# ouguangjun/Leg-KILO

Measured on AMD Instinct MI355X. Metric: LiDAR scans/sec (per-point ESKF update), 100k-pt scan, higher is better.
Workload: dtype f64

## Files before the change

leg-kilo_amd/csrc/lk_map_kernels.h:

```cpp
#pragma once
#include "lk_device.h"
#include "lk_eig3.h"

#define LK_MB 256

__device__ __forceinline__ void wave_fence() {
    __builtin_amdgcn_fence(__ATOMIC_RELEASE, "workgroup");
    __builtin_amdgcn_fence(__ATOMIC_ACQUIRE, "workgroup");
}
__device__ __forceinline__ int bcast0(int v) { return __builtin_amdgcn_readfirstlane(v); }
__device__ __forceinline__ int wave_min_i(int v) {
#pragma unroll
    for (int o = 32; o > 0; o >>= 1) {
        int t = __shfl_xor(v, o, LK_WAVE);
        v = t < v ? t : v;
    }
    return v;
}

template <int N>
__device__ __forceinline__ void wave_sum_n(double* v) {
    const int lane = threadIdx.x & 63;
    constexpr int H5 = (N + 1) / 2, H4 = (H5 + 1) / 2, H3 = (H4 + 1) / 2, H2 = (H3 + 1) / 2, H1 = (H2 + 1) / 2, H0 = (H1 + 1) / 2;
    auto step = [&](const int n, const int half, const int mask) {
        const bool hi = (lane & mask) != 0;
#pragma unroll
        for (int j = 0; j < half; ++j) {
            const double a = v[j];
            const double b = (half + j < n) ? v[half + j] : 0.0;
            const double send = hi ? a : b, keep = hi ? b : a;
            v[j] = keep + __shfl_xor(send, mask, LK_WAVE);
        }
    };
    step(N, H5, 32);
    step(H5, H4, 16);
    step(H4, H3, 8);
    step(H3, H2, 4);
    step(H2, H1, 2);
    step(H1, H0, 1);
    double r[N];
#pragma unroll
    for (int c = 0; c < N; ++c) {
        int rem = c, src = 0;
        if (rem >= H5) rem -= H5, src |= 32;
        if (rem >= H4) rem -= H4, src |= 16;
        if (rem >= H3) rem -= H3, src |= 8;
        if (rem >= H2) rem -= H2, src |= 4;
        if (rem >= H1) rem -= H1, src |= 2;
        if (rem >= H0) rem -= H0, src |= 1;
        r[c] = __shfl(v[0], src, LK_WAVE);
    }
#pragma unroll
    for (int c = 0; c < N; ++c) v[c] = r[c];
}

struct PtU {
    double pw[3];
    double var[6];
};

__device__ __forceinline__ void load_pt(const lk_pt_rec* base, const int* idx, int j, double* pw, double* var) {
    const lk_pt_rec* r = &base[idx ? idx[j] : j];
#pragma unroll
    for (int c = 0; c < 3; ++c) pw[c] = r->pw[c];
#pragma unroll
    for (int c = 0; c < 6; ++c) var[c] = r->var[c];
}

__device__ __forceinline__ void eig_sym3_cols_dev(const double* Ain, double* ev, double* v0, double* v1, double* v2) {
    lk_eig_sym3_cols(Ain, ev, v0, v1, v2);
}

__device__ __noinline__ bool dev_init_plane(lk_plane_rec* pl, lk_match_rec* mr, float planer_threshold, const lk_pt_rec* base,
                                            const int* idx, int count) {
    const int lane = threadIdx.x & 63;
    double s[9];
#pragma unroll
    for (int q = 0; q < 9; ++q) s[q] = 0.0;
    for (int j = lane; j < count; j += LK_WAVE) {
        double pw[3], var[6];
        load_pt(base, idx, j, pw, var);
        s[0] += pw[0], s[1] += pw[1], s[2] += pw[2];
        s[3] += pw[0] * pw[0], s[4] += pw[0] * pw[1], s[5] += pw[0] * pw[2];
        s[6] += pw[1] * pw[1], s[7] += pw[1] * pw[2], s[8] += pw[2] * pw[2];
    }
#pragma unroll
    for (int q = 0; q < 9; ++q) s[q] = wave_sum(s[q]);
    const double n = (double)count;
    double c[3] = {s[0] / n, s[1] / n, s[2] / n};
    double cov[6] = {s[3] / n - c[0] * c[0], s[4] / n - c[0] * c[1], s[5] / n - c[0] * c[2],
                     s[6] / n - c[1] * c[1], s[7] / n - c[1] * c[2], s[8] / n - c[2] * c[2]};
    double ev[3], V0[3], V1[3], V2[3];
    eig_sym3_cols_dev(cov, ev, V0, V1, V2);
    int imin = 0, imax = 0;
    {
        double lo = ev[0], hi = ev[0];
        if (ev[1] < lo) imin = 1, lo = ev[1];
        if (ev[1] > hi) imax = 1, hi = ev[1];
        if (ev[2] < lo) imin = 2, lo = ev[2];
        if (ev[2] > hi) imax = 2, hi = ev[2];
    }
    int imid = 3 - imin - imax;
    if (imid > 2) imid = imin;
    const bool is_plane = ev[imin] < (double)planer_threshold;
    double acc[21];
#pragma unroll
    for (int q = 0; q < 21; ++q) acc[q] = 0.0;
    auto col = [&](int k, double* o) {
        o[0] = (k == 0) ? V0[0] : (k == 1) ? V1[0] : V2[0];
        o[1] = (k == 0) ? V0[1] : (k == 1) ? V1[1] : V2[1];
        o[2] = (k == 0) ? V0[2] : (k == 1) ? V1[2] : V2[2];
    };
    auto evk = [&](int k) { return (k == 0) ? ev[0] : (k == 1) ? ev[1] : ev[2]; };
    double vmin[3], vmid[3], vmax[3];
    col(imin, vmin), col(imid, vmid), col(imax, vmax);
    const double emin = evk(imin), emid = evk(imid), emax = evk(imax);
    if (is_plane) {
        double rhsA[9], rhsB[9];
#pragma unroll
        for (int r = 0; r < 3; ++r)
#pragma unroll
            for (int cc = 0; cc < 3; ++cc) {
                rhsA[3 * r + cc] = vmid[r] * vmin[cc] + vmin[r] * vmid[cc];
                rhsB[3 * r + cc] = vmax[r] * vmin[cc] + vmin[r] * vmax[cc];
            }
        const double denA = count * (emin - emid), denB = count * (emin - emax);
        const double invn = 1.0 / count;
        for (int j = lane; j < count; j += LK_WAVE) {
            double pw[3], var[6];
            load_pt(base, idx, j, pw, var);
            double q[3] = {pw[0] - c[0], pw[1] - c[1], pw[2] - c[2]};
            double la[3] = {q[0] / denA, q[1] / denA, q[2] / denA};
            double lb[3] = {q[0] / denB, q[1] / denB, q[2] / denB};
            double FA[3], FB[3];
#pragma unroll
            for (int cc = 0; cc < 3; ++cc) {
                FA[cc] = la[0] * rhsA[cc] + la[1] * rhsA[3 + cc] + la[2] * rhsA[6 + cc];
                FB[cc] = lb[0] * rhsB[cc] + lb[1] * rhsB[3 + cc] + lb[2] * rhsB[6 + cc];
            }
            double J[6][3];
#pragma unroll
            for (int r = 0; r < 3; ++r)
#pragma unroll
                for (int cc = 0; cc < 3; ++cc) {
                    J[r][cc] = vmid[r] * FA[cc] + vmax[r] * FB[cc];
                    J[3 + r][cc] = (r == cc) ? invn : 0.0;
                }
            double Sv[3][3] = {{var[0], var[1], var[2]}, {var[1], var[3], var[4]}, {var[2], var[4], var[5]}};
            double JV[6][3];
#pragma unroll
            for (int r = 0; r < 6; ++r)
#pragma unroll
                for (int cc = 0; cc < 3; ++cc) JV[r][cc] = J[r][0] * Sv[0][cc] + J[r][1] * Sv[1][cc] + J[r][2] * Sv[2][cc];
            int k = 0;
#pragma unroll
// ... 1258 lines not shown
        }
        r.state |= LK_NODE_INIT_OCTO;
        r.new_points = 0;
    }
    if (keep && r.npts > 0) {
        if (r.npts <= LK_BLOCK_PTS) {
            r.block = alloc_block(m);
            for (int j = lane; j < r.npts; j += LK_WAVE) m.blocks[r.block].pts[j] = bpts[idx_in[begin + j]];
        } else {
            r.state |= LK_NODE_PTS_DROPPED;
        }
    }
    node_store(nd, r);
}

#ifdef LK_KERNELS_ELSEWHERE
__global__ void __launch_bounds__(LK_MB)
    lk_build_tree_kernel(LkMap map, LkParams pr, const lk_pt_rec* __restrict__ bpts, int* idxA, int* idxB);
#else
__global__ void __launch_bounds__(LK_MB)
    lk_build_tree_kernel(LkMap map, LkParams pr, const lk_pt_rec* __restrict__ bpts, int* idxA, int* idxB) {
    const int wave = (blockIdx.x * LK_MB + threadIdx.x) >> 6;
    const int nwaves = (gridDim.x * LK_MB) >> 6;
    const int n_touched = (int)map.counters[LK_CTR_TOUCHED];
    for (int t = wave; t < n_touched; t += nwaves) {
        const int root = bcast0(map.touched[t]);
        const int b = bcast0((int)map.nodes[root].pad_[1]), e = bcast0((int)map.nodes[root].pad_[2]);
        dev_build_node<0>(map, pr, root, bpts, idxA, idxB, b, e - b);
    }
}
#endif

__device__ __forceinline__ void dev_bucket_begin(const LkMap& map) {
    __shared__ int base, nfreed;
    if (threadIdx.x == 0) {
        int fc = (int)map.counters[LK_CTR_FREE];
        base = fc > 0 ? fc : 0;
        unsigned int nf = map.counters[LK_CTR_FREED];
        nfreed = (int)(nf < map.max_blocks ? nf : map.max_blocks);
        if (base + nfreed > (int)map.max_blocks) nfreed = (int)map.max_blocks - base;
        map.counters[LK_CTR_TOUCHED] = 0;
        map.counters[LK_CTR_SCRATCH] = 0;
        map.counters[LK_CTR_HEAVY] = 0;
        map.counters[LK_CTR_GROUPS] = 0;
        map.counters[LK_CTR_GIDX] = 0;
        map.counters[LK_CTR_FALLBACK] = 0;
    }
    __syncthreads();
    for (int i = threadIdx.x; i < nfreed; i += (int)blockDim.x) map.free_list[base + i] = map.freed_next[i];
    __syncthreads();
    if (threadIdx.x == 0) {
        map.counters[LK_CTR_FREE] = (unsigned int)(base + nfreed);
        map.counters[LK_CTR_FREED] = 0;
    }
}
#ifdef LK_KERNELS_ELSEWHERE
__global__ void __launch_bounds__(256) lk_bucket_begin_kernel(LkMap map);
#else
__global__ void __launch_bounds__(256) lk_bucket_begin_kernel(LkMap map) { dev_bucket_begin(map); }
#endif
__device__ __forceinline__ void dev_bucket_begin_wave(const LkMap& map) {
    const int lane = threadIdx.x & 63;
    int base = 0, nfreed = 0;
    if (lane == 0) {
        const int fc = (int)map.counters[LK_CTR_FREE];
        base = fc > 0 ? fc : 0;
        const unsigned int nf = map.counters[LK_CTR_FREED];
        nfreed = (int)(nf < map.max_blocks ? nf : map.max_blocks);
        if (base + nfreed > (int)map.max_blocks) nfreed = (int)map.max_blocks - base;
        map.counters[LK_CTR_TOUCHED] = 0;
        map.counters[LK_CTR_SCRATCH] = 0;
        map.counters[LK_CTR_HEAVY] = 0;
        map.counters[LK_CTR_GROUPS] = 0;
        map.counters[LK_CTR_GIDX] = 0;
        map.counters[LK_CTR_FALLBACK] = 0;
    }
    base = bcast0(base), nfreed = bcast0(nfreed);
    for (int i = lane; i < nfreed; i += LK_WAVE) map.free_list[base + i] = map.freed_next[i];
    wave_fence();
    if (lane == 0) {
        map.counters[LK_CTR_FREE] = (unsigned int)(base + nfreed);
        map.counters[LK_CTR_FREED] = 0;
    }
    wave_fence();
}
__device__ __forceinline__ void dev_stamp_dirty_roots(const LkMap& map, const LkParams& pr, int n_touched) {
    const int lane = threadIdx.x & 63;
    for (int t = lane; t < n_touched; t += LK_WAVE) {
        const int root = map.touched[t];
        const lk_node_rec* nd = &map.nodes[root];
        if (!root_is_light(pr, (int)nd->pad_[0], nd->state, map.planes[root].flags, nd->npts, nd->new_points)) map.dirty[root] = map.epoch;
    }
}

#ifdef LK_KERNELS_ELSEWHERE
__global__ void __launch_bounds__(256) lk_pool_init_kernel(LkMap map, unsigned int n_hash);
#else
__global__ void __launch_bounds__(256) lk_pool_init_kernel(LkMap map, unsigned int n_hash) {
    const unsigned int i = blockIdx.x * 256 + threadIdx.x;
    if (i < n_hash) map.hash[i] = make_int4((int)0x80000000, (int)0x80000000, (int)0x80000000, LK_EMPTY);
    if (i < map.max_nodes) {
        lk_node_rec* nd = &map.nodes[i];
        for (int c = 0; c < 8; ++c) nd->child[c] = -1;
        nd->voxel_center[0] = nd->voxel_center[1] = nd->voxel_center[2] = 0.0;
        nd->quater_length = 0.f;
        nd->layer = 0, nd->npts = 0, nd->new_points = 0, nd->state = 0, nd->block = -1;
        nd->key[0] = nd->key[1] = nd->key[2] = 0;
        nd->list_head = -1;
        for (int c = 0; c < 8; ++c) nd->pad_[c] = 0;
        map.planes[i].flags = 0;
        map.match[i].flags = 0;
    }
    if (i < LK_CTR_COUNT) map.counters[i] = 0;
}
#endif

#ifdef LK_KERNELS_ELSEWHERE
__global__ void __launch_bounds__(256) lk_grid_bounds_kernel(LkMap map, unsigned int n_hash, int* __restrict__ mm );
#else
__global__ void __launch_bounds__(256) lk_grid_bounds_kernel(LkMap map, unsigned int n_hash, int* __restrict__ mm ) {
    const unsigned int i = blockIdx.x * 256 + threadIdx.x;
    int lo[3] = {INT_MAX, INT_MAX, INT_MAX}, hi[3] = {INT_MIN, INT_MIN, INT_MIN};
    if (i < n_hash) {
        const int4 e = map.hash[i];
        if (e.w >= 0) lo[0] = hi[0] = e.x, lo[1] = hi[1] = e.y, lo[2] = hi[2] = e.z;
    }
#pragma unroll
    for (int c = 0; c < 3; ++c) {
#pragma unroll
        for (int o = 32; o > 0; o >>= 1) {
            lo[c] = min(lo[c], __shfl_xor(lo[c], o, LK_WAVE));
            hi[c] = max(hi[c], __shfl_xor(hi[c], o, LK_WAVE));
        }
    }
    if ((threadIdx.x & 63) == 0 && lo[0] <= hi[0]) {
        atomicMin(&mm[0], lo[0]), atomicMin(&mm[1], lo[1]), atomicMin(&mm[2], lo[2]);
        atomicMax(&mm[3], hi[0]), atomicMax(&mm[4], hi[1]), atomicMax(&mm[5], hi[2]);
    }
}
#endif
#ifdef LK_KERNELS_ELSEWHERE
__global__ void __launch_bounds__(256) lk_grid_fill_kernel(LkMap map, unsigned int n_hash, int max_layer, unsigned int* __restrict__ cursor,
                                                           unsigned int cand_end);
#else
__global__ void __launch_bounds__(256) lk_grid_fill_kernel(LkMap map, unsigned int n_hash, int max_layer, unsigned int* __restrict__ cursor,
                                                           unsigned int cand_end) {
    const unsigned int i = blockIdx.x * 256 + threadIdx.x;
    if (i >= n_hash) return;
    const int4 e = map.hash[i];
    if (e.w < 0) return;
    const size_t c = ((size_t)(e.z - map.gmin[2]) * (size_t)map.gdim[1] + (size_t)(e.y - map.gmin[1])) * (size_t)map.gdim[0] + (size_t)(e.x - map.gmin[0]);
    lk_match_rec r = map.match[e.w];
    r.pad_ = (unsigned int)e.w;
    if (!(r.flags & LK_PLANE_IS_PLANE)) {
        unsigned int first = 0, count = 0;
        for (int pass = 0; pass < 2; ++pass) {
            if (pass == 1) {
                if (count == 0) break;
                first = atomicAdd(cursor, count);
                if (first + count > cand_end) {
                    atomicExch(cursor + 1, 1u);
                    count = 0;
                    break;
                }
            }
            unsigned int k = 0;
            int stack_node[LK_MAX_LAYER + 1], stack_ci[LK_MAX_LAYER + 1];
            int level = 0;
            stack_node[0] = e.w, stack_ci[0] = 0;
            while (level >= 0) {
                const int node = stack_node[level];
                if (stack_ci[level] == 0 && level > 0) {
                    const unsigned int fl = map.match[node].flags;
                    if (fl & LK_PLANE_IS_PLANE) {
                        if (pass == 1) {
                            lk_match_rec cr = map.match[node];
                            cr.pad_ = (unsigned int)node;
                            map.match[first + k] = cr;
                        }
                        ++k;
                        --level;
                        continue;
                    }
                }
                if (level >= max_layer || level >= LK_MAX_LAYER) {
                    --level;
                    continue;
                }
                int child = -1;
                while (stack_ci[level] < 8 && child < 0) child = map.nodes[node].child[stack_ci[level]++];
                if (child >= 0) {
                    ++level;
                    stack_node[level] = child, stack_ci[level] = 0;
                } else {
                    --level;
                }
            }
            if (pass == 0) count = k;
        }
        r.flags = LK_GRID_LIST;
        unsigned int fc[2] = {first, count};
        memcpy(&r.center[0], fc, sizeof(fc));
    }
    map.match[map.grid_base + c] = r;
}
#endif

#ifdef LK_KERNELS_ELSEWHERE
__global__ void __launch_bounds__(256) lk_derive_match_kernel(LkMap map, int n);
#else
__global__ void __launch_bounds__(256) lk_derive_match_kernel(LkMap map, int n) {
    const int i = blockIdx.x * 256 + threadIdx.x;
    if (i >= n) return;
    if (map.planes[i].flags & LK_PLANE_IS_PLANE)
        lk_derive_match(&map.planes[i], &map.match[i]);
    else
        map.match[i].flags = map.planes[i].flags;
}
#endif

#ifdef LK_KERNELS_ELSEWHERE
__global__ void __launch_bounds__(256) lk_hash_insert_kernel(LkMap map, LkParams pr, const lk_root_rec* __restrict__ roots, int n);
#else
__global__ void __launch_bounds__(256) lk_hash_insert_kernel(LkMap map, LkParams pr, const lk_root_rec* __restrict__ roots, int n) {
    const int i = blockIdx.x * 256 + threadIdx.x;
    if (i >= n) return;
    unsigned int s = lk_hash3(roots[i].key[0], roots[i].key[1], roots[i].key[2]) & map.hash_mask;
    int* slotw = reinterpret_cast<int*>(map.hash);
    for (unsigned int trips = 0; trips <= map.hash_mask; ++trips) {
        if (atomicCAS(&slotw[4 * s + 3], LK_EMPTY, roots[i].node) == LK_EMPTY) {
            slotw[4 * s + 0] = roots[i].key[0];
            slotw[4 * s + 1] = roots[i].key[1];
            slotw[4 * s + 2] = roots[i].key[2];
            return;
        }
        s = (s + 1) & map.hash_mask;
    }
    atomicOr(&map.counters[LK_CTR_ERR], LK_E_HASH_FULL);
}
#endif

struct LkSlideBox {
    int x_max, x_min, y_max, y_min, z_max, z_min;
};

#ifdef LK_KERNELS_ELSEWHERE
__global__ void __launch_bounds__(256)
    lk_slide_mark_kernel(LkMap map, LkSlideBox box, unsigned int n_hash, unsigned int* __restrict__ alive_node,
                         unsigned int* __restrict__ alive_block, lk_root_rec* __restrict__ kept,
                         unsigned int* __restrict__ cnt );
#else
__global__ void __launch_bounds__(256)
    lk_slide_mark_kernel(LkMap map, LkSlideBox box, unsigned int n_hash, unsigned int* __restrict__ alive_node,
                         unsigned int* __restrict__ alive_block, lk_root_rec* __restrict__ kept,
                         unsigned int* __restrict__ cnt ) {
    const unsigned int i = blockIdx.x * 256 + threadIdx.x;
    if (i >= n_hash) return;
    const int4 e = map.hash[i];
    if (e.w < 0) return;
    const bool should_remove = e.x > box.x_max || e.x < box.x_min || e.y > box.y_max || e.y < box.y_min ||
                               e.z > box.z_max || e.z < box.z_min;
    if (should_remove) {
        atomicAdd(&cnt[1], 1u);
        return;
    }
    const unsigned int k = atomicAdd(&cnt[0], 1u);
    kept[k].key[0] = e.x, kept[k].key[1] = e.y, kept[k].key[2] = e.z;
    kept[k].node = e.w;
    int st_node[LK_MAX_LAYER + 2], st_ci[LK_MAX_LAYER + 2];
    int depth = 0;
    st_node[0] = e.w, st_ci[0] = 0;
    alive_node[e.w] = 1u;
    {
        const int b = map.nodes[e.w].block;
        if (b >= 0) alive_block[b] = 1u;
    }
    while (depth >= 0) {
        const int ci = st_ci[depth];
        if (ci == 8) {
            --depth;
            continue;
        }
        st_ci[depth] = ci + 1;
        const int child = map.nodes[st_node[depth]].child[ci];
        if (child < 0) continue;
        alive_node[child] = 1u;
        const int b = map.nodes[child].block;
        if (b >= 0) alive_block[b] = 1u;
        if (depth + 1 < LK_MAX_LAYER + 2) {
            ++depth;
            st_node[depth] = child, st_ci[depth] = 0;
        }
    }
}
#endif

#ifdef LK_KERNELS_ELSEWHERE
__global__ void __launch_bounds__(256)
    lk_slide_move_nodes_kernel(LkMap map, unsigned int n_nodes, const unsigned int* __restrict__ alive_node,
                               const unsigned int* __restrict__ new_node, const unsigned int* __restrict__ new_block,
                               lk_node_rec* __restrict__ tn, lk_plane_rec* __restrict__ tp, lk_match_rec* __restrict__ tm);
#else
__global__ void __launch_bounds__(256)
    lk_slide_move_nodes_kernel(LkMap map, unsigned int n_nodes, const unsigned int* __restrict__ alive_node,
                               const unsigned int* __restrict__ new_node, const unsigned int* __restrict__ new_block,
                               lk_node_rec* __restrict__ tn, lk_plane_rec* __restrict__ tp, lk_match_rec* __restrict__ tm) {
    const unsigned int i = blockIdx.x * 256 + threadIdx.x;
    if (i >= n_nodes || !alive_node[i]) return;
    const unsigned int j = new_node[i];
    lk_node_rec r = map.nodes[i];
#pragma unroll
    for (int c = 0; c < 8; ++c)
        if (r.child[c] >= 0) r.child[c] = (int)new_node[r.child[c]];
    if (r.block >= 0) r.block = (int)new_block[r.block];
    r.list_head = -1;
    r.pad_[0] = 0;
    tn[j] = r;
    tp[j] = map.planes[i];
    tm[j] = map.match[i];
}
#endif

#ifdef LK_KERNELS_ELSEWHERE
__global__ void __launch_bounds__(64)
    lk_slide_move_blocks_kernel(LkMap map, const unsigned int* __restrict__ alive_block,
                                const unsigned int* __restrict__ new_block, lk_block_rec* __restrict__ tb);
#else
__global__ void __launch_bounds__(64)
    lk_slide_move_blocks_kernel(LkMap map, const unsigned int* __restrict__ alive_block,
                                const unsigned int* __restrict__ new_block, lk_block_rec* __restrict__ tb) {
// ... 41 lines not shown
```

leg-kilo_amd/csrc/lk_point_kernels.h:

```cpp
#pragma once
#include "lk_device.h"

#define LK_PB 256
#define LK_ROWS_STORE(v, p) __builtin_nontemporal_store((v), (p))
#define LK_RB 64

struct Match {
    double* row;
    float lazy_d;
    double lazy_sig;
};

struct RecTail {
    double2 v0, v1, v2, v3, v4;
};
template <bool XID, bool PRE = false>
__device__ __forceinline__ void eval_plane(const lk_match_rec* __restrict__ mr, double2 q0, double2 q1, double2 q2,
                                           float pd, float pradius, int node, int layer, const PointLite& g,
                                           const BucketConst& bc, const LkParams& pr, bool& success, double& prob,
                                           Match& best, const RecTail* pre = nullptr) {
    const double2* sv = reinterpret_cast<const double2*>(mr->s11);
    double2 v0, v1, v2, v3, v4;
    if (PRE) v0 = pre->v0, v1 = pre->v1, v2 = pre->v2, v3 = pre->v3, v4 = pre->v4;
    else v0 = sv[0], v1 = sv[1], v2 = sv[2], v3 = sv[3], v4 = sv[4];
    V3 c = V3{q0.x, q0.y, q1.x}, n = V3{q1.y, q2.x, q2.y};
    double sd = dot3(n.x, g.p_w.x, n.y, g.p_w.y, n.z, g.p_w.z) + (double)pd;
    float dis_to_plane = (float)fabs(sd);
    float dis_to_center = (float)((c.x - g.p_w.x) * (c.x - g.p_w.x) + (c.y - g.p_w.y) * (c.y - g.p_w.y) +
                                  (c.z - g.p_w.z) * (c.z - g.p_w.z));
    float range_dis = sqrtf(dis_to_center - dis_to_plane * dis_to_plane);
    if (!((double)range_dis <= 3.0 * (double)pradius)) return;
    const V3 q = V3{g.p_w.x - c.x, g.p_w.y - c.y, g.p_w.z - c.z};
    const S3 s11 = S3{v0.x, v0.y, v1.x, v1.y, v2.x, v2.y};
    const double sig_pl = quad3(s11, q) - 2.0 * dot3(q.x, v3.x, q.y, v3.y, q.z, v4.x) + v4.y;
    const PlaneTerms t = plane_terms<XID>(g, bc, pr, n);
    const double sig_r = sig_pl + t.ta;
    const double sigma_l = sig_r + (quad3(bc.Prr, t.w) + quad3(bc.Ppp, n));
    const double d2 = (double)dis_to_plane * (double)dis_to_plane;
    if (!(d2 < (pr.sigma_num * pr.sigma_num) * sigma_l)) return;
    bool take;
    if (!success) {
        take = true;
        prob = -1.0;
        best.lazy_d = dis_to_plane;
        best.lazy_sig = sigma_l;
    } else {
        if (prob < 0.0)
            prob = 1.0 / (sqrt(best.lazy_sig)) * exp(-0.5 * (double)best.lazy_d * (double)best.lazy_d / best.lazy_sig);
        const double this_prob = 1.0 / sqrt(sigma_l) * exp(-0.5 * d2 / sigma_l);
        take = this_prob > prob;
        if (take) prob = this_prob;
    }
    success = true;
    if (take) {
        double* r = best.row;
        r[0] = t.w.x, r[1] = t.w.y, r[2] = t.w.z;
        r[3] = n.x, r[4] = n.y, r[5] = n.z;
        r[6] = -(double)(float)sd;
        const double Rv = pr.lidar_ratio * sig_r;
        const double ri = lk_inv_nodecision(Rv);
        r[7] = t.w.x * ri, r[8] = t.w.y * ri, r[9] = t.w.z * ri;
        r[10] = n.x * ri, r[11] = n.y * ri, r[12] = n.z * ri;
        r[13] = Rv;
        r[14] = 1.0;
    }
}

template <bool XID>
__device__ __forceinline__ bool match_root(const LkMap& m, int root, const bool grid_cell, const PointLite& g,
                                           const BucketConst& bc, const LkParams& pr, bool& success, double& prob, Match& best) {
    const int max_layer = pr.max_layer;
    int n0 = root, n1 = -1, n2 = -1, n3 = -1, n4 = -1;
    unsigned int cis = 0;
    int level = 0;
    bool fresh = true;
    while (level >= 0) {
        int node = (level == 0) ? n0 : (level == 1) ? n1 : (level == 2) ? n2 : (level == 3) ? n3 : n4;
        if (fresh) {
            const lk_match_rec* pl = &m.match[node];
            const double2* q = reinterpret_cast<const double2*>(pl);
            double2 q0 = q[0], q1 = q[1], q2 = q[2];
            float4 tail = *reinterpret_cast<const float4*>(&pl->d);
            RecTail rt;
            rt.v0 = q[4], rt.v1 = q[5], rt.v2 = q[6], rt.v3 = q[7], rt.v4 = q[8];
            pin_chunk(q0), pin_chunk(q1), pin_chunk(q2), pin_chunk(tail);
            pin_chunk(rt.v0), pin_chunk(rt.v1), pin_chunk(rt.v2), pin_chunk(rt.v3), pin_chunk(rt.v4);
            if (grid_cell && level == 0) {
                const unsigned int id = __float_as_uint(tail.w);
                if (id == LK_GRID_EMPTY) return false;
                n0 = node = (int)id;
            }
            if (__float_as_uint(tail.z) & LK_PLANE_IS_PLANE) {
                eval_plane<XID, true>(pl, q0, q1, q2, tail.x, tail.y, node, level, g, bc, pr, success, prob, best, &rt);
                --level;
                fresh = false;
                continue;
            }
            if (level >= max_layer || level >= LK_MAX_LAYER) {
                --level;
                fresh = false;
                continue;
            }
            cis &= ~(15u << (4 * level));
        }
        const int4* ch = reinterpret_cast<const int4*>(m.nodes[node].child);
        int4 ca = ch[0], cb = ch[1];
        pin_chunk(ca), pin_chunk(cb);
        unsigned int ci = (cis >> (4 * level)) & 15u;
        int child = -1;
        while (ci < 8u && child < 0) {
            child = (ci == 0) ? ca.x : (ci == 1) ? ca.y : (ci == 2) ? ca.z : (ci == 3) ? ca.w
                  : (ci == 4) ? cb.x : (ci == 5) ? cb.y : (ci == 6) ? cb.z : cb.w;
            ++ci;
        }
        cis = (cis & ~(15u << (4 * level))) | (ci << (4 * level));
        if (child >= 0) {
            ++level;
            if (level == 1) n1 = child;
            else if (level == 2) n2 = child;
            else if (level == 3) n3 = child;
            else n4 = child;
            fresh = true;
        } else {
            --level;
            fresh = false;
        }
    }
    return true;
}

template <bool XID>
__device__ __forceinline__ bool match_flat(const LkMap& m, int cell, const PointLite& g, const BucketConst& bc, const LkParams& pr,
                                           bool& success, double& prob, Match& best) {
    int idx = cell, remaining = 1;
    bool header = true;
    while (remaining > 0) {
        const lk_match_rec* pl = &m.match[idx];
        const double2* q = reinterpret_cast<const double2*>(pl);
        double2 q0 = q[0], q1 = q[1], q2 = q[2];
        float4 tail = *reinterpret_cast<const float4*>(&pl->d);
        RecTail rt;
        rt.v0 = q[4], rt.v1 = q[5], rt.v2 = q[6], rt.v3 = q[7], rt.v4 = q[8];
        pin_chunk(q0), pin_chunk(q1), pin_chunk(q2), pin_chunk(tail);
        pin_chunk(rt.v0), pin_chunk(rt.v1), pin_chunk(rt.v2), pin_chunk(rt.v3), pin_chunk(rt.v4);
        const unsigned int fl = __float_as_uint(tail.z);
        if (header) {
            header = false;
            if (__float_as_uint(tail.w) == LK_GRID_EMPTY) return false;
            if (!(fl & LK_PLANE_IS_PLANE)) {
                idx = (int)(unsigned int)__double_as_longlong(q0.x);
                remaining = (int)(unsigned int)(__double_as_longlong(q0.x) >> 32);
                continue;
            }
        }
        eval_plane<XID, true>(pl, q0, q1, q2, tail.x, tail.y, 0, 0, g, bc, pr, success, prob, best, &rt);
        ++idx;
        --remaining;
    }
    return true;
}

template <int GRID>
__device__ __forceinline__ int find_root(const LkMap& m, int kx, int ky, int kz) {
    if (GRID == 1 || (GRID == 2 && m.grid_on)) {
        const unsigned int ux = (unsigned int)(kx - m.gmin[0]), uy = (unsigned int)(ky - m.gmin[1]), uz = (unsigned int)(kz - m.gmin[2]);
        if (ux >= (unsigned int)m.gdim[0] || uy >= (unsigned int)m.gdim[1] || uz >= (unsigned int)m.gdim[2]) return -1;
        return (int)(m.grid_base + (uz * (unsigned int)m.gdim[1] + uy) * (unsigned int)m.gdim[0] + ux);
    }
    return hash_find(m, kx, ky, kz);
}

struct LkOvView {
    const unsigned long long* keys;
    unsigned int hash_mask;
    const lk_match_rec* match;
    const lk_node_rec* nodes;
    const unsigned int* bits;
};
__device__ __forceinline__ int find_root_ov(const LkMap& base, const LkOvView& ov, int kx, int ky, int kz) {
    const unsigned int ux = (unsigned int)(kx - base.gmin[0]), uy = (unsigned int)(ky - base.gmin[1]), uz = (unsigned int)(kz - base.gmin[2]);
    const bool in = ux < (unsigned int)base.gdim[0] && uy < (unsigned int)base.gdim[1] && uz < (unsigned int)base.gdim[2];
    unsigned int cell = 0;
    if (in) {
        cell = (uz * (unsigned int)base.gdim[1] + uy) * (unsigned int)base.gdim[0] + ux;
        if (!((ov.bits[cell >> 5] >> (cell & 31u)) & 1u)) return (int)(base.grid_base + cell);
    }
    const int lim = 1 << 20;
    if (!(kx < -lim || kx >= lim || ky < -lim || ky >= lim || kz < -lim || kz >= lim)) {
        const unsigned long long pk = ((unsigned long long)((unsigned int)kx & 0x1fffffu)) | ((unsigned long long)((unsigned int)ky & 0x1fffffu) << 21) |
                                      ((unsigned long long)((unsigned int)kz & 0x1fffffu) << 42);
        unsigned int s = lk_hash3(kx, ky, kz) & ov.hash_mask;
        for (unsigned int probe = 0; probe <= ov.hash_mask; probe += 2) {
            const unsigned long long e0 = ov.keys[s], e1 = ov.keys[(s + 1) & ov.hash_mask];
            if (e0 == pk) return -2 - (int)s;
            if (e0 == 0x8000000000000000ull) break;
            if (e1 == pk) return -2 - (int)((s + 1) & ov.hash_mask);
            if (e1 == 0x8000000000000000ull) break;
            s = (s + 2) & ov.hash_mask;
        }
    }
    return in ? (int)(base.grid_base + cell) : -1;
}

__device__ __forceinline__ void neighbour_key(const LkParams& pr, const float* loc, const int* key, int* near) {
    const double vs = (double)pr.voxel_size_f;
    const double ql = (double)(pr.voxel_size_f / 4);
#pragma unroll
    for (int j = 0; j < 3; ++j) {
        const double vc = (0.5 + key[j]) * vs;
        near[j] = key[j];
        if ((double)loc[j] > (vc + ql))
            near[j] += 1;
        else if ((double)loc[j] < (vc - ql))
            near[j] -= 1;
    }
}

struct ResidualOut {
    double* h6;
    double* rows8 = nullptr;
    double* z;
    double* R;
    unsigned char* valid;
    float* world;
    int2* ids;
    int2* ids_lane = nullptr;
    int xmap_slots = 0;
    const lk_point* alt_pts = nullptr;
    const unsigned long long* alt_use = nullptr;
};
#define LK_SPEC_NONE ((int)0x80000000)
__device__ __forceinline__ int spec_code(int root, const int* key) {
    return root >= 0 ? root : ~(int)(lk_hash3(key[0], key[1], key[2]) & LK_NEWROOT_MASK);
}
__device__ __forceinline__ bool spec_suspect(const LkMap& m, int code, unsigned int from) {
    if (code == LK_SPEC_NONE) return false;
    const unsigned int stamp = code >= 0 ? m.dirty[code] : m.newroot[~code];
    return stamp >= from;
}

#define LK_ROW2 15

#if LK_OPT_WAVES
#define LK_RES_BOUNDS __launch_bounds__(LK_RB, LK_OPT_WAVES)
#else
#define LK_RES_BOUNDS __launch_bounds__(LK_RB)
#endif
template <bool EMIT_ROWS, int GRID = 2, bool XID = false, bool SHORT = false, bool SPEC = false>
__device__ __forceinline__ double residual_tile(const LkMap& map, const LkParams& pr, const BucketConst& bc,
                                                const float4* __restrict__ spts, int i, int n, double* rows, int lane,
                                                const ResidualOut& out, size_t out_base, const LkOvView* ovv = nullptr) {
    bool ok = false;
    double h[6] = {0, 0, 0, 0, 0, 0}, z = 0, R = 0;
    {
        PointLite g;
        int root = -1, nroot = -1;
        if (i < n) {
            typedef float lk_f4v __attribute__((ext_vector_type(4)));
            const lk_f4v p = __builtin_nontemporal_load(reinterpret_cast<const lk_f4v*>(spts) + i);
            g = point_lite<XID>(p.x, p.y, p.z, bc, pr);
            if (out.world) {
                float4 w = make_float4((float)g.p_w.x, (float)g.p_w.y, (float)g.p_w.z, 0.f);
                reinterpret_cast<float4*>(out.world + out_base * 4)[i] = w;
            }
            float loc[3];
            int key[3];
            key_trunc(g.p_w, pr, loc, key);
            root = GRID == 3 ? find_root_ov(map, *ovv, key[0], key[1], key[2]) : find_root<GRID>(map, key[0], key[1], key[2]);
            if (SPEC) {
                if (out.ids_lane) *out.ids_lane = make_int2(spec_code(root, key), LK_SPEC_NONE);
                else out.ids[out_base + i] = make_int2(spec_code(root, key), LK_SPEC_NONE);
            }
        }
        bool success = false;
        double prob = 0;
        Match best;
        best.row = rows + lane * LK_ROW2;
        const bool grid_cell = GRID == 1 || GRID == 3 || (GRID == 2 && map.grid_on != 0);
        bool home = false;
        LkMap pmv = {};
        if (GRID == 3) pmv.match = const_cast<lk_match_rec*>(ovv->match), pmv.nodes = const_cast<lk_node_rec*>(ovv->nodes);
        if (root >= 0) home = grid_cell ? match_flat<XID>(map, root, g, bc, pr, success, prob, best) : match_root<XID>(map, root, false, g, bc, pr, success, prob, best);
        else if (GRID == 3 && root <= -2) home = match_root<XID>(pmv, -2 - root, false, g, bc, pr, success, prob, best);
        if (home && !success) {
            float loc[3];
            int key[3], near[3];
            key_trunc(g.p_w, pr, loc, key);
            neighbour_key(pr, loc, key, near);
            if (near[0] != key[0] || near[1] != key[1] || near[2] != key[2]) {
                nroot = GRID == 3 ? find_root_ov(map, *ovv, near[0], near[1], near[2]) : find_root<GRID>(map, near[0], near[1], near[2]);
                if (SPEC) {
                    if (out.ids_lane) out.ids_lane->y = spec_code(nroot, near);
                    else out.ids[out_base + i].y = spec_code(nroot, near);
                }
            }
            if (nroot >= 0) {
                if (grid_cell) match_flat<XID>(map, nroot, g, bc, pr, success, prob, best);
                else match_root<XID>(map, nroot, false, g, bc, pr, success, prob, best);
            } else if (GRID == 3 && nroot <= -2) {
                match_root<XID>(pmv, -2 - nroot, false, g, bc, pr, success, prob, best);
            }
        }
        ok = success;
    }
    if (!ok) {
        double* r = rows + lane * LK_ROW2;
#pragma unroll
        for (int a = 0; a < LK_ROW2; ++a) r[a] = 0.0;
    }
    __builtin_amdgcn_fence(__ATOMIC_RELEASE, "wavefront");
    __builtin_amdgcn_wave_barrier();
    __builtin_amdgcn_fence(__ATOMIC_ACQUIRE, "wavefront");
    if (EMIT_ROWS) {
        typedef double lk_d2v __attribute__((ext_vector_type(2)));
        const int tile0 = i - lane;
        const int nv = n - tile0 < 64 ? n - tile0 : 64;
        const size_t o0 = out_base + (size_t)tile0;
        if (out.rows8) {
            lk_d2v* dst = reinterpret_cast<lk_d2v*>(out.rows8 + o0 * 8);
#pragma unroll
            for (int k = 0; k < 4; ++k) {
                const int e = k * 64 + lane, row = e >> 2, c = (e & 3) * 2;
                if (row < nv) {
                    const double* r = rows + row * LK_ROW2;
                    lk_d2v v;
                    v.x = r[c], v.y = c == 6 ? r[13] : r[c + 1];
                    LK_ROWS_STORE(v, dst + e);
                }
            }
        } else {
            lk_d2v* dst = reinterpret_cast<lk_d2v*>(out.h6 + o0 * 6);
#pragma unroll
            for (int k = 0; k < 3; ++k) {
                const int e = k * 64 + lane, row = e / 3, c = (e - row * 3) * 2;
                if (row < nv) {
                    lk_d2v v;
                    v.x = rows[row * LK_ROW2 + c], v.y = rows[row * LK_ROW2 + c + 1];
                    LK_ROWS_STORE(v, dst + e);
                }
            }
            if (lane < nv) {
                const double* r = rows + lane * LK_ROW2;
                LK_ROWS_STORE(r[6], out.z + o0 + lane);
                LK_ROWS_STORE(r[13], out.R + o0 + lane);
            }
        }
        if (lane < nv) LK_ROWS_STORE((unsigned char)(rows[lane * LK_ROW2 + 14] != 0.0 ? 1 : 0), out.valid + o0 + lane);
        return 0.0;
    }
    const int q = lane & 31, half = lane >> 5;
    const unsigned long long tw = (q < 8) ? 0x2818574737271707ull : (q < 16) ? 0x3a59493929584838ull : (q < 24) ? 0x6968675c5b4b5a4aull : 0xeeeeeeeeed6c6b6aull;
    const unsigned int ab = (unsigned int)(tw >> ((q & 7) * 8)) & 0xffu;
    const int a = (int)(ab & 15u), b = (int)(ab >> 4);
    const double* base = rows + (half * 32) * LK_ROW2;
    double acc = 0.0;
    if (SHORT) {
        const int nv = __builtin_amdgcn_readfirstlane(n - (i - lane));
        const int jm = nv >= 32 ? 32 : ((nv + 7) & ~7);
        for (int j0 = 0; j0 < jm; j0 += 8) {
#pragma unroll
            for (int j = 0; j < 8; ++j) {
                const double* r = base + (j0 + j) * LK_ROW2;
                acc = __builtin_fma(r[a], r[b], acc);
            }
        }
    } else {
#pragma unroll
        for (int j = 0; j < 32; ++j) {
            const double* r = base + j * LK_ROW2;
            acc = __builtin_fma(r[a], r[b], acc);
        }
    }
    acc += __shfl_xor(acc, 32, LK_WAVE);
    return acc;
}

template <bool EMIT_ROWS, int GRID = 0, bool XID = false, bool SPEC = false>
__global__ void LK_RES_BOUNDS
    lk_residual_kernel(LkMap map, LkParams pr, const LkFilter* __restrict__ filters, const lk_point* __restrict__ pts,
                       size_t pts_slot_stride, int n, double* __restrict__ partials, size_t part_slot_stride,
                       ResidualOut out, size_t out_slot_stride) {
    __shared__ double stage[LK_RB / LK_WAVE][64 * LK_ROW2];
    int slot = blockIdx.y, bx = blockIdx.x;
    if (out.xmap_slots > 0) {
        const unsigned int T = (unsigned int)((n + LK_RB - 1) / LK_RB), c = (T + 7u) >> 3;
        const unsigned int x = blockIdx.x & 7u, j = blockIdx.x >> 3;
        const unsigned int t = x * c + j % c;
        slot = (int)(j / c);
        if (t >= T || slot >= out.xmap_slots) return;
        bx = (int)t;
    }
    const int tid = threadIdx.x;
    const int lane = tid & 63, wv = tid >> 6;
    BucketConst bc;
    load_bucket_const<false>(&filters[slot], pr, bc);
    if (out.alt_use && out.alt_use[1] != 0ull) pts = out.alt_pts;
    const double acc = residual_tile<EMIT_ROWS, GRID, XID, false, SPEC>(map, pr, bc, reinterpret_cast<const float4*>(pts + (size_t)slot * pts_slot_stride),
                                                bx * LK_RB + tid, n, &stage[wv][0], lane, out, (size_t)slot * out_slot_stride);
    if (!EMIT_ROWS && lane < LK_NPART) {
        const size_t wave_id = (size_t)bx * (LK_RB / LK_WAVE) + wv;
        partials[(size_t)slot * part_slot_stride + wave_id * LK_NPART + lane] = (lane < 29) ? acc : 0.0;
    }
}

__device__ __forceinline__ void spec_wait(const LkMap& m, int word, unsigned int need) {
    if (need != 0 && (threadIdx.x & 63) == 0) {
        const unsigned long long t0 = wall_clock64();
        while (__hip_atomic_load(&m.spec[word], __ATOMIC_ACQUIRE, __HIP_MEMORY_SCOPE_AGENT) < need) {
            __builtin_amdgcn_s_sleep(4);
            if (wall_clock64() - t0 > 20000000ull) {
                atomicOr(&m.counters[LK_CTR_ERR], LK_E_SPEC_TIMEOUT);
                break;
            }
        }
    }
    __builtin_amdgcn_fence(__ATOMIC_ACQUIRE, "agent");
}
template <bool XID>
__global__ void LK_RES_BOUNDS
    lk_verify_kernel(LkMap map, LkParams pr, const LkFilter* __restrict__ filters, const lk_point* __restrict__ pts, int n,
                     double* __restrict__ partials, ResidualOut out, unsigned int dirty_from, unsigned int need_done) {
    __shared__ double stage[64 * LK_ROW2];
    const int lane = threadIdx.x;
    const int i = blockIdx.x * LK_RB + lane;
    bool susp = false;
    if (i < n) {
        const int2 c = out.ids[i];
        susp = spec_suspect(map, c.x, dirty_from) || spec_suspect(map, c.y, dirty_from);
    }
    if (__ballot(susp) == 0ull) return;
    if (lane == 0) atomicAdd(&map.counters[LK_CTR_SPEC_REDO], 1u);
    spec_wait(map, LK_SPEC_DONE, need_done);
    BucketConst bc;
    load_bucket_const<false>(&filters[0], pr, bc);
    const double acc = residual_tile<false, 0, XID>(map, pr, bc, reinterpret_cast<const float4*>(pts), i, n, stage, lane, out, (size_t)0);
    if (lane < LK_NPART) partials[(size_t)blockIdx.x * LK_NPART + lane] = (lane < 29) ? acc : 0.0;
}

template <int GRID>
__global__ void LK_RES_BOUNDS
    lk_residual_ragged_kernel(LkMap map, LkParams pr, const LkFilter* __restrict__ filters, const lk_point* __restrict__ pts,
                              LkRagged rg, int b, double* __restrict__ partials, size_t part_slot_stride) {
    __shared__ double stage[LK_RB / LK_WAVE][64 * LK_ROW2];
    const int slot = blockIdx.y;
    if (b >= rag_nb(rg, slot)) return;
    const unsigned long long* po = rag_pt_off(rg, slot);
    const unsigned long long base = po[b];
    const int n = (int)(po[b + 1] - base);
    if ((int)(blockIdx.x * LK_RB) >= n) return;
    const int tid = threadIdx.x;
    const int lane = tid & 63, wv = tid >> 6;
    BucketConst bc;
    load_bucket_const<false>(&filters[slot], pr, bc);
    ResidualOut out;
    out.h6 = nullptr, out.z = nullptr, out.R = nullptr, out.valid = nullptr, out.world = nullptr;
    const double acc = residual_tile<false, GRID>(map, pr, bc, reinterpret_cast<const float4*>(pts + base), blockIdx.x * LK_RB + tid, n,
                                            &stage[wv][0], lane, out, (size_t)0);
    if (lane < LK_NPART) {
        const size_t wave_id = (size_t)blockIdx.x * (LK_RB / LK_WAVE) + wv;
        partials[(size_t)slot * part_slot_stride + wave_id * LK_NPART + lane] = (lane < 29) ? acc : 0.0;
    }
}

__device__ __forceinline__ int root_find_or_create(const LkMap& m, const LkParams& pr, const int* key) {
    {
        int r = hash_find(m, key[0], key[1], key[2]);
        if (r >= 0) return r;
    }
    unsigned int s = lk_hash3(key[0], key[1], key[2]) & m.hash_mask;
    int* slotw = reinterpret_cast<int*>(m.hash);
    for (unsigned int trips = 0; trips < 64u * (m.hash_mask + 1u); ++trips) {
        int w = __hip_atomic_load(&slotw[4 * s + 3], __ATOMIC_ACQUIRE, __HIP_MEMORY_SCOPE_AGENT);
        if (w == LK_EMPTY) {
            int expected = LK_EMPTY;
            if (__hip_atomic_compare_exchange_strong(&slotw[4 * s + 3], &expected, LK_LOCKED, __ATOMIC_ACQ_REL,
                                                     __ATOMIC_ACQUIRE, __HIP_MEMORY_SCOPE_AGENT)) {
                unsigned int id = atomicAdd(&m.counters[LK_CTR_NODES], 1u);
                if (id >= m.max_nodes) {
                    atomicOr(&m.counters[LK_CTR_ERR], LK_E_NODES_FULL);
                    __hip_atomic_store(&slotw[4 * s + 3], LK_EMPTY, __ATOMIC_RELEASE, __HIP_MEMORY_SCOPE_AGENT);
                    return -1;
                }
                atomicAdd(&m.counters[LK_CTR_ROOTS], 1u);
                lk_node_rec* nd = &m.nodes[id];
                double vs = (double)pr.voxel_size_f;
#pragma unroll
                for (int c = 0; c < 8; ++c) nd->child[c] = -1;
#pragma unroll
                for (int c = 0; c < 3; ++c) {
                    nd->voxel_center[c] = (0.5 + key[c]) * vs;
                    nd->key[c] = key[c];
                }
                nd->quater_length = pr.voxel_size_f / 4;
                nd->layer = 0;
                nd->npts = 0;
                nd->new_points = 0;
                nd->state = LK_NODE_UPDATE_ENABLE;
                nd->block = -1;
                nd->list_head = -1;
                nd->pad_[0] = 0;
                m.planes[id].flags = 0;
                m.match[id].flags = 0;
                m.dirty[id] = m.epoch;
                m.newroot[lk_hash3(key[0], key[1], key[2]) & LK_NEWROOT_MASK] = m.epoch;
                slotw[4 * s + 0] = key[0];
                slotw[4 * s + 1] = key[1];
                slotw[4 * s + 2] = key[2];
                __hip_atomic_store(&slotw[4 * s + 3], (int)id, __ATOMIC_RELEASE, __HIP_MEMORY_SCOPE_AGENT);
                return (int)id;
            }
            continue;
        }
        if (w == LK_LOCKED) {
            __builtin_amdgcn_s_sleep(1);
            continue;
        }
        int kx = __hip_atomic_load(&slotw[4 * s + 0], __ATOMIC_RELAXED, __HIP_MEMORY_SCOPE_AGENT);
        int ky = __hip_atomic_load(&slotw[4 * s + 1], __ATOMIC_RELAXED, __HIP_MEMORY_SCOPE_AGENT);
        int kz = __hip_atomic_load(&slotw[4 * s + 2], __ATOMIC_RELAXED, __HIP_MEMORY_SCOPE_AGENT);
        if (kx == key[0] && ky == key[1] && kz == key[2]) return w;
        s = (s + 1) & m.hash_mask;
    }
    atomicOr(&m.counters[LK_CTR_ERR], LK_E_HASH_FULL);
    return -1;
}

// ... 77 lines not shown
```

Baseline: 670,700.

## Precompute squared range bound in grid records; use permlane32 swap for half-wave reduction

When building the dense grid, each plane record's radius is replaced by a precomputed float bound on the squared range. The grid-path plane test can then compare range² directly, with no sqrtf or double conversion in the per-point hot loop. The bound is built with careful float rounding so it keeps the original decision exactly. Separately, the 32-lane cross-half shuffle in the row reduction is replaced with permlane32_swap on the two 32-bit halves. The risk is that any other reader of the grid copy's radius field now sees a changed meaning.

Result: faster. 689,100 (median of 6 runs) (+2.7%).

```diff
diff --git a/leg-kilo_amd/csrc/lk_map_kernels.h b/leg-kilo_amd/csrc/lk_map_kernels.h
--- a/leg-kilo_amd/csrc/lk_map_kernels.h
+++ b/leg-kilo_amd/csrc/lk_map_kernels.h
@@ -1,6 +1,7 @@
 #pragma once
 #include "lk_device.h"
 #include "lk_eig3.h"
+#include "lk_range_bound.h"
 
 #define LK_MB 256
 
@@ -1565,6 +1566,7 @@
     const size_t c = ((size_t)(e.z - map.gmin[2]) * (size_t)map.gdim[1] + (size_t)(e.y - map.gmin[1])) * (size_t)map.gdim[0] + (size_t)(e.x - map.gmin[0]);
     lk_match_rec r = map.match[e.w];
     r.pad_ = (unsigned int)e.w;
+    r.radius = lk_range_bound(r.radius);
     if (!(r.flags & LK_PLANE_IS_PLANE)) {
         unsigned int first = 0, count = 0;
         for (int pass = 0; pass < 2; ++pass) {
@@ -1589,6 +1591,7 @@
                         if (pass == 1) {
                             lk_match_rec cr = map.match[node];
                             cr.pad_ = (unsigned int)node;
+                            cr.radius = lk_range_bound(cr.radius);
                             map.match[first + k] = cr;
                         }
                         ++k;
diff --git a/leg-kilo_amd/csrc/lk_point_kernels.h b/leg-kilo_amd/csrc/lk_point_kernels.h
--- a/leg-kilo_amd/csrc/lk_point_kernels.h
+++ b/leg-kilo_amd/csrc/lk_point_kernels.h
@@ -14,7 +14,7 @@
 struct RecTail {
     double2 v0, v1, v2, v3, v4;
 };
-template <bool XID, bool PRE = false>
+template <bool XID, bool PRE = false, bool BOUND = false>
 __device__ __forceinline__ void eval_plane(const lk_match_rec* __restrict__ mr, double2 q0, double2 q1, double2 q2,
                                            float pd, float pradius, int node, int layer, const PointLite& g,
                                            const BucketConst& bc, const LkParams& pr, bool& success, double& prob,
@@ -28,8 +28,13 @@
     float dis_to_plane = (float)fabs(sd);
     float dis_to_center = (float)((c.x - g.p_w.x) * (c.x - g.p_w.x) + (c.y - g.p_w.y) * (c.y - g.p_w.y) +
                                   (c.z - g.p_w.z) * (c.z - g.p_w.z));
-    float range_dis = sqrtf(dis_to_center - dis_to_plane * dis_to_plane);
-    if (!((double)range_dis <= 3.0 * (double)pradius)) return;
+    const float range2 = dis_to_center - dis_to_plane * dis_to_plane;
+    if (BOUND) {
+        if (!(range2 >= 0.f && range2 <= pradius)) return;
+    } else {
+        float range_dis = sqrtf(range2);
+        if (!((double)range_dis <= 3.0 * (double)pradius)) return;
+    }
     const V3 q = V3{g.p_w.x - c.x, g.p_w.y - c.y, g.p_w.z - c.z};
     const S3 s11 = S3{v0.x, v0.y, v1.x, v1.y, v2.x, v2.y};
     const double sig_pl = quad3(s11, q) - 2.0 * dot3(q.x, v3.x, q.y, v3.y, q.z, v4.x) + v4.y;
@@ -153,7 +158,7 @@
                 continue;
             }
         }
-        eval_plane<XID, true>(pl, q0, q1, q2, tail.x, tail.y, 0, 0, g, bc, pr, success, prob, best, &rt);
+        eval_plane<XID, true, true>(pl, q0, q1, q2, tail.x, tail.y, 0, 0, g, bc, pr, success, prob, best, &rt);
         ++idx;
         --remaining;
     }
@@ -371,7 +376,12 @@
             acc = __builtin_fma(r[a], r[b], acc);
         }
     }
-    acc += __shfl_xor(acc, 32, LK_WAVE);
+    {
+        const unsigned int lo = (unsigned int)__double2loint(acc), hi = (unsigned int)__double2hiint(acc);
+        const lk_u2 l = __builtin_amdgcn_permlane32_swap(lo, lo, false, false);
+        const lk_u2 h = __builtin_amdgcn_permlane32_swap(hi, hi, false, false);
+        acc = __hiloint2double((int)h.x, (int)l.x) + __hiloint2double((int)h.y, (int)l.y);
+    }
     return acc;
 }
 
diff --git a/leg-kilo_amd/csrc/lk_range_bound.h b/leg-kilo_amd/csrc/lk_range_bound.h
--- /dev/null
+++ b/leg-kilo_amd/csrc/lk_range_bound.h
@@ -0,0 +1,38 @@
+#pragma once
+#include <stdint.h>
+
+#if defined(__HIPCC__)
+#define LK_RANGE_FN __host__ __device__ __forceinline__
+#else
+#define LK_RANGE_FN static inline
+#endif
+
+LK_RANGE_FN uint32_t lk_range_f2u(float v) {
+    uint32_t u;
+    __builtin_memcpy(&u, &v, sizeof(u));
+    return u;
+}
+LK_RANGE_FN float lk_range_u2f(uint32_t u) {
+    float v;
+    __builtin_memcpy(&v, &u, sizeof(v));
+    return v;
+}
+
+LK_RANGE_FN float lk_range_bound(float radius) {
+    const double flt_max = 3.4028234663852886e38;
+    const double T = 3.0 * (double)radius;
+    if (T != T) return radius;
+    if (T < 0.0) return -1.0f;
+    if (T == 0.0) return 0.0f;
+    if (T > flt_max) return T > 1.7976931348623157e308 ? radius : 3.4028234663852886e38f;
+    float f = (float)T;
+    if ((double)f > T) f = lk_range_u2f(lk_range_f2u(f) - 1u);
+    const uint32_t fu = lk_range_f2u(f);
+    const double up = fu == 0x7f7fffffu ? 3.4028236692093846e38  : (double)lk_range_u2f(fu + 1u);
+    const double m = 0.5 * ((double)f + up);
+    const double B = m * m;
+    if (B > flt_max) return 3.4028234663852886e38f;
+    float c = (float)B;
+    if ((double)c >= B) c = lk_range_u2f(lk_range_f2u(c) - 1u);
+    return c;
+}
```
